# glgerard/MDBN

Hardware: AMD Instinct MI355X
Metric: CD-k Gibbs steps/sec (samples/sec), GRBM 4096->1024 CD-1 (higher is better)
Workload: dtype f32; 1 GPU; GRBM 4096->1024 CD-1, batch 512 per GPU, fp32, N(0,1) rows resident in HBM (BASELINE configs[1]); global_batch=512, k=1, n_data=32768, parallelism=dp1

## Files before the change

### include/mdbn_hip.h

```cpp
#ifndef MDBN_HIP_H
#define MDBN_HIP_H

#include <stddef.h>
#include <stdint.h>

#ifdef __cplusplus
extern "C" {
#endif

#define MDBN_OK       0
#define MDBN_EINVAL  (-1)
#define MDBN_EHIP    (-2)
#define MDBN_ENOSPC  (-3)

#define MDBN_VERSION 2

typedef struct mdbn_ctx mdbn_ctx;

typedef struct mdbn_rng {
    uint64_t seed;
    uint32_t stream_id;
    uint32_t step;
    uint32_t draw;
    uint32_t reserved;
// ... 49 lines not shown
    float batch_size;
    float n_rows;
    float cost_scale;
    float *cost_out;
    void *W_planes;
    int32_t phase;
    int32_t reserved;
} mdbn_update_args;

int  mdbn_version(void);
int  mdbn_last_error(char *buf, size_t n);
int  mdbn_source_hash(char *buf, size_t n);

int  mdbn_ctx_create(mdbn_ctx **out, int device);
int  mdbn_ctx_destroy(mdbn_ctx *ctx);

int  mdbn_bal_segment(int32_t tiles, int32_t stages, int32_t workgroups, int32_t w, int32_t k, int32_t *out);
int  mdbn_set_option(mdbn_ctx *ctx, const char *name, int64_t value);

int  mdbn_kernel_timing(mdbn_ctx *ctx, int enable);
int  mdbn_kernel_timing_read(mdbn_ctx *ctx, int64_t *n_launches, double *total_ms);
int  mdbn_kernel_timing_detail(mdbn_ctx *ctx, int64_t cap, double *ms, double *alg_flop,
                               double *pipe_flop, int32_t *kind, int64_t *n_launches);

int  mdbn_workspace_bytes(int64_t B, int64_t V, int64_t H, int64_t *bytes);
int  mdbn_workspace_bytes_ctx(mdbn_ctx *ctx, int64_t B, int64_t V, int64_t H, int64_t *bytes);
int  mdbn_padded_ld(int64_t cols, int64_t *ld);
int  mdbn_planes_bytes(int64_t B, int64_t ldv, int64_t ldh, int64_t *bytes);
int  mdbn_planes_alt_bytes(int64_t B, int64_t ldv, int64_t *bytes);
int  mdbn_ahead_bytes_ctx(mdbn_ctx *ctx, int64_t B, int64_t V, int64_t H, int64_t ldv, int64_t ldh, int64_t *bytes);
int  mdbn_planes_eligible(int64_t B, int64_t V, int64_t H, int64_t ldv, int64_t ldh, int32_t *eligible);
int  mdbn_planes_eligible_ctx(mdbn_ctx *ctx, int64_t B, int64_t V, int64_t H, int64_t ldv, int64_t ldh, int32_t *eligible);
int  mdbn_split_planes(mdbn_ctx *ctx, void *stream, const float *x, int64_t rows, int64_t ld, void *planes);
int  mdbn_stats_floats(int64_t V, int64_t ldv, int64_t ldh, int64_t *n);

int  mdbn_gather_rows(mdbn_ctx *ctx, void *stream, const float *src, int64_t n_rows,
                      int64_t cols, int64_t ld_src, const void *indexes, int index_is_64,
                      int64_t n_idx, float *dst, int64_t ld_dst);

int  mdbn_gather_rows_host(mdbn_ctx *ctx, void *stream, const float *src, int64_t n_rows,
                           int64_t cols, int64_t ld_src, const void *indexes, int index_is_64,
                           int64_t n_idx, float *dst, int64_t ld_dst, int workgroups, int threads);

int  mdbn_host_gather_rows(const float *table, int64_t n_rows, int64_t cols, int64_t ld,
                           const int64_t *indexes, int64_t n, float *out, int64_t ld_out, int threads);

// ... 193 lines not shown
```

### mdbn_amd/_lib.py

```python
import ctypes as C
import os

HERE = os.path.dirname(os.path.abspath(__file__))
LIB_PATH = os.path.join(HERE, "libmdbn_hip.so")


class MdbnError(RuntimeError):
    pass


class Rng(C.Structure):
    _fields_ = [("seed", C.c_uint64), ("stream_id", C.c_uint32), ("step", C.c_uint32),
                ("draw", C.c_uint32), ("reserved", C.c_uint32), ("row_offset", C.c_uint64)]


class _Sized(C.Structure):

    def __init__(self, *a, **kw):
        super(_Sized, self).__init__(*a, **kw)
        self.struct_size = C.sizeof(type(self))


class CdArgs(_Sized):
    _fields_ = [("struct_size", C.c_uint64), ("data", C.c_void_p), ("n_data", C.c_int64), ("indexes", C.c_void_p),
# ... 17 lines not shown
                ("vbias", C.c_void_p), ("vbias_speed", C.c_void_p),
                ("V", C.c_int64), ("H", C.c_int64), ("ldv", C.c_int64), ("ldh", C.c_int64),
                ("stats", C.c_void_p),
                ("lr", C.c_float), ("lambda_1", C.c_float), ("lambda_2", C.c_float),
                ("weightcost", C.c_float), ("momentum", C.c_float),
                ("batch_size", C.c_float), ("n_rows", C.c_float),
                ("cost_scale", C.c_float), ("cost_out", C.c_void_p), ("W_planes", C.c_void_p),
                ("phase", C.c_int32), ("reserved", C.c_int32)]


_i64, _i32, _f32, _vp = C.c_int64, C.c_int, C.c_float, C.c_void_p
_rngp = C.POINTER(Rng)

SIGNATURES = {
    "mdbn_version": [],
    "mdbn_last_error": [C.c_char_p, C.c_size_t],
    "mdbn_source_hash": [C.c_char_p, C.c_size_t],
    "mdbn_ctx_create": [C.POINTER(_vp), _i32],
    "mdbn_ctx_destroy": [_vp],
    "mdbn_set_option": [_vp, C.c_char_p, _i64],
    "mdbn_bal_segment": [_i32, _i32, _i32, _i32, _i32, C.POINTER(_i32)],
    "mdbn_kernel_timing": [_vp, _i32],
    "mdbn_kernel_timing_read": [_vp, C.POINTER(_i64), C.POINTER(C.c_double)],
    "mdbn_kernel_timing_detail": [_vp, _i64, C.POINTER(C.c_double), C.POINTER(C.c_double),
                                  C.POINTER(C.c_double), C.POINTER(C.c_int32), C.POINTER(_i64)],
    "mdbn_workspace_bytes": [_i64, _i64, _i64, C.POINTER(_i64)],
    "mdbn_workspace_bytes_ctx": [_vp, _i64, _i64, _i64, C.POINTER(_i64)],
    "mdbn_padded_ld": [_i64, C.POINTER(_i64)],
    "mdbn_planes_bytes": [_i64, _i64, _i64, C.POINTER(_i64)],
    "mdbn_planes_alt_bytes": [_i64, _i64, C.POINTER(_i64)],
    "mdbn_ahead_bytes_ctx": [_vp, _i64, _i64, _i64, _i64, _i64, C.POINTER(_i64)],
    "mdbn_planes_eligible": [_i64, _i64, _i64, _i64, _i64, C.POINTER(_i32)],
    "mdbn_planes_eligible_ctx": [_vp, _i64, _i64, _i64, _i64, _i64, C.POINTER(_i32)],
    "mdbn_split_planes": [_vp, _vp, _vp, _i64, _i64, _vp],
    "mdbn_stats_floats": [_i64, _i64, _i64, C.POINTER(_i64)],
    "mdbn_gather_rows": [_vp, _vp, _vp, _i64, _i64, _i64, _vp, _i32, _i64, _vp, _i64],
    "mdbn_gather_rows_host": [_vp, _vp, _vp, _i64, _i64, _i64, _vp, _i32, _i64, _vp, _i64, _i32, _i32],
    "mdbn_host_gather_rows": [_vp, _i64, _i64, _i64, _vp, _i64, _vp, _i64, _i32],
    "mdbn_feeder_create": [_vp, _vp, _i64, _i64, _i64, _i64, _i32, C.POINTER(_vp), _i64, _i32, C.POINTER(_vp)],
    "mdbn_feeder_submit": [_vp, _vp, _i64, C.POINTER(_i64)],
    "mdbn_feeder_acquire": [_vp, _i64, _vp, C.POINTER(_i32)],
    "mdbn_feeder_release": [_vp, _i64, _vp],
    "mdbn_feeder_stats": [_vp, C.POINTER(C.c_double)],
    "mdbn_feeder_cancel": [_vp],
    "mdbn_feeder_destroy": [_vp],
    "mdbn_propup_sample": [_vp, _vp, _vp, _i64, _i64, _vp, _i64, _i64, _i64, _vp,
# ... 125 lines not shown
```

### mdbn_amd/csrc/mdbn_capi.hip

```cpp
#include <hip/hip_runtime.h>
#include <algorithm>
#include <cstdint>
#include <initializer_list>
#include <cstdarg>
#include <cstdio>
#include <cstring>
#include <string>
#include <utility>
#include <vector>
#include "mdbn_capi_internal.h"
#include "mdbn_kernels.h"
#include "mdbn_small.h"
#include "mdbn_thin.h"
#include "mdbn_gchain.h"

using namespace mdbn;
using namespace mdbn::capi;

static const Options g_default_options;
static GemmTiming g_no_timing;
static thread_local const Options* t_opt = &g_default_options;
static thread_local GemmTiming* t_timing = &g_no_timing;
#define g_timing (*t_timing)

namespace mdbn {
namespace capi {
CtxScope::CtxScope(mdbn_ctx* c) : prev_opt(t_opt), prev_timing(t_timing)
{
// ... 82 lines not shown
    return p;
}

bool prefer_skinny(int64_t M, int64_t N, int64_t K)
{
    if (!g_opt_skinny_gemm) return false;
    if (M <= 64) return true;
    if (K > g_opt_skinny_fused_max_k) return false;
    const int64_t tiles_m = (M + 63) / 64, strips = (N + 31) / 32;
    if (K > 64 * tiles_m * strips) return false;
    return M * N * K <= (K <= 512 ? 3 : 1) * g_opt_skinny_max_macs;
}


#define g_opt_gemm_bf16x6 (t_opt->gemm_bf16x6)
#define g_opt_small_fused (t_opt->small_fused)
#define g_opt_thin_fused (t_opt->thin_fused)
#define g_opt_gchain (t_opt->gchain)
#define g_opt_gemm_planes (t_opt->gemm_planes)
#define g_opt_planes_mfma (t_opt->planes_mfma)
#define g_opt_early_w (t_opt->early_w)
#define g_opt_narrow_tiles (t_opt->narrow_tiles)
#define g_opt_slab_tail (t_opt->slab_tail)
#define g_opt_feed_copy_streams (t_opt->feed_copy_streams)
#define g_opt_gather_ahead (t_opt->gather_ahead)
#define g_opt_bf16_inputs (t_opt->bf16_inputs)
#define g_opt_planes_min_work (t_opt->planes_min_work)
#define g_opt_comm_cus (t_opt->comm_cus)
#define g_opt_bal_blocks (t_opt->bal_blocks)
constexpr int kMaxBalBlocks = 256;

bool try_bf16x6(Plan& p, int64_t M, int64_t N, int64_t K, bool unsplit = false)
{
    if (p.skinny || K < 64) return false;
    const int64_t tm = (M + 127) / 128, tn = (N + 127) / 128, tiles = tm * tn;
    int64_t sk = 1;
    if (!unsplit) {
        sk = std::min(std::max<int64_t>(1, kTargetJobs / tiles), std::max<int64_t>(1, K / kMinSplitK));
    } else if (p.splitk != 1) {
        return false;
    }
    if (tiles * sk < g_opt_x6_min_jobs) return false;
    int64_t kchunk = ((K + sk - 1) / sk + 31) / 32 * 32;
    sk = (K + kchunk - 1) / kchunk;
    p.x6 = 1;
    p.bn = 128; p.bk = 32; p.cw = 1;
// ... 220 lines not shown
                      const unsigned short* Wp, int64_t V, int64_t H, int64_t ncols, int64_t rows, EpiArgs e, bool want_cost,
                      const Workspace& ws, hipStream_t s, int* n_cost_out)
{
    const int64_t Kdim = dir == 0 ? V : H, Ndim = dir == 0 ? H : V;
    PlaneGemmArgs g{};
    g.A = A; g.lda = lda; g.pa = pa; g.ap = ap;
    g.B = Wp; g.ldb = H; g.pb = V * H;
    g.M = (int)rows; g.N = (int)Ndim; g.K = (int)Kdim;
    g.tiles_m = (int)(rows / 128); g.tiles_n = (int)(Ndim / 128);
    {
        const Plan p = plan_forward(rows, Ndim, Kdim, e.ld, false);
        g.splitk = p.splitk; g.kchunk = p.kchunk;
    }
    int bal = bal_blocks(ctx, comm_cus, (int64_t)g.tiles_m * g.tiles_n, Kdim / 32), bal_slabs = 0;
    if (bal) {
        bal_slabs = bal_max_segments(g.tiles_m * g.tiles_n, (int)(Kdim / 32), bal);
        if ((int64_t)bal_slabs * rows * e.ld > ws.slab_floats) bal = 0;
        if ((int64_t)bal_slabs * rows * e.ld * 4 >= (int64_t)1 << 31) bal = 0;
    }
    if (!bal && g_opt_narrow_tiles && g_opt_fused_epilogue && dir == 1 && g.splitk == 2 && Ndim % 64 == 0 && g_opt_planes_mfma == 16 &&
        !g_opt_bf16_inputs && (ap == 1 || ap == 3) && (int64_t)g.tiles_m * (Ndim / 64) <= 2 * ctx->num_cu &&
        (!e.target || (e.ld_target % 4 == 0 && ((uintptr_t)e.target & 15) == 0))) {
        g.bn = 64; g.tiles_n = (int)(Ndim / 64); g.splitk = 1; g.kchunk = (int)Kdim;
    }
    const bool fuse = !bal && g_opt_fused_epilogue && g.splitk == 1;
    const int nb = fuse ? g.tiles_m * g.tiles_n : epilogue_blocks(rows, e.ld);
    e.rows = (int)rows; e.cols = (int)ncols;
    e.cost_partials = nullptr;
    if (want_cost) {
        if (nb > ws.cost_floats) return fail(MDBN_ENOSPC, "cost scratch exhausted");
        e.cost_partials = ws.cost_partials;
        if (n_cost_out) *n_cost_out = nb;
    }
    const int lb = dir == 0 ? LAY_MN : LAY_K;
    if (bal) {
        g.bal = bal; g.fused = 0; g.C = ws.slabs; g.ldc = e.ld; g.slab_stride = rows * e.ld;
        g.xcd_group = bal >= 4 * g.tiles_m * g.tiles_n ? 0 : 1;
        g.splitk = 1; g.kchunk = (int)Kdim; g.c_bytes = (int64_t)bal_slabs * rows * e.ld * 4;
        e.slabs = ws.slabs; e.slab_stride = g.slab_stride; e.nsplit = bal_slabs;
        e.bal_P = bal; e.bal_S = (int)(Kdim / 32); e.bal_tiles_m = g.tiles_m; e.bal_tiles_n = g.tiles_n;
        {
            const int tiles = g.tiles_m * g.tiles_n;
            bool uniform = true;
            for (int t = 0; t < tiles && uniform; ++t) uniform = bal_tile_slabs(t, tiles, e.bal_S, bal) == bal_slabs;
            if (uniform) e.bal_P = 0;
        }
// ... 366 lines not shown
    return MDBN_OK;
}

int mdbn_last_error(char* buf, size_t n)
{
    if (!buf || n == 0) return MDBN_EINVAL;
    snprintf(buf, n, "%s", g_err.c_str());
    return MDBN_OK;
}

int mdbn_ctx_create(mdbn_ctx** out, int device)
{
    REQUIRE(out != nullptr, "out is NULL");
    int count = 0;
    HIP_OK(hipGetDeviceCount(&count));
    REQUIRE(device >= 0 && device < count, "device %d out of range (%d visible)", device, count);
    hipDeviceProp_t prop;
    HIP_OK(hipGetDeviceProperties(&prop, device));
    if (strncmp(prop.gcnArchName, "gfx950", 6) != 0)
        return fail(MDBN_EHIP, "device %d is %s; this library is built for gfx950 only", device, prop.gcnArchName);
    mdbn_ctx* c = new mdbn_ctx;
    c->device = device;
    c->num_cu = prop.multiProcessorCount;
    *out = c;
    return MDBN_OK;
}

int mdbn_ctx_destroy(mdbn_ctx* ctx)
{
    CtxScope ctx_scope(ctx);
    if (ctx) {
        if (ctx->ev_fork) (void)hipEventDestroy(ctx->ev_fork);
        if (ctx->ev_join) (void)hipEventDestroy(ctx->ev_join);
        if (ctx->side) (void)hipStreamDestroy(ctx->side);
        if (ctx->comm) (void)mdbn_comm_destroy(ctx);
        if (ctx->gc_flags) (void)hipFree(ctx->gc_flags);
    }
    delete ctx;
    return MDBN_OK;
}

#ifdef MDBN_STAMP
int mdbn_debug_set_stamps(void* p) { g_stamps = (unsigned long long*)p; return MDBN_OK; }
#endif

int mdbn_bal_segment(int32_t tiles, int32_t stages, int32_t workgroups, int32_t w, int32_t k, int32_t* out)
// ... 162 lines not shown
        return MDBN_OK;
    }
    if (strcmp(name, "fused_update") == 0) {
        ctx->opt.fused_update = value != 0;
        return MDBN_OK;
    }
    if (strcmp(name, "fused_epilogue") == 0) {
        ctx->opt.fused_epilogue = value != 0;
        return MDBN_OK;
    }
    if (strcmp(name, "update_overlap") == 0) {
        ctx->opt.update_overlap = value != 0;
        return MDBN_OK;
    }
    return fail(MDBN_EINVAL, "unknown option %s", name);
}

int mdbn_kernel_timing(mdbn_ctx* ctx, int enable)
{
    CtxScope ctx_scope(ctx);
    REQUIRE(ctx != nullptr, "ctx is NULL");
    g_timing.enabled = enable != 0;
    g_timing.used = 0;
    return MDBN_OK;
}

int mdbn_kernel_timing_read(mdbn_ctx* ctx, int64_t* n_launches, double* total_ms)
{
    CtxScope ctx_scope(ctx);
    REQUIRE(ctx && n_launches && total_ms, "NULL argument");
    double tot = 0.0;
    for (size_t i = 0; i < g_timing.used; ++i) {
        HIP_OK(hipEventSynchronize(g_timing.pool[i].second));
        float ms = 0.f;
        HIP_OK(hipEventElapsedTime(&ms, g_timing.pool[i].first, g_timing.pool[i].second));
        tot += ms;
    }
    *n_launches = (int64_t)g_timing.used;
    *total_ms = tot;
    return MDBN_OK;
}

int mdbn_kernel_timing_detail(mdbn_ctx* ctx, int64_t cap, double* ms, double* alg_flop, double* pipe_flop,
                              int32_t* kind, int64_t* n_launches)
{
    CtxScope ctx_scope(ctx);
// ... 809 lines not shown
```

### mdbn_amd/csrc/mdbn_capi_internal.h

```cpp
#pragma once
#include <hip/hip_runtime.h>
#include <cstdint>
#include <utility>
#include <vector>
#include "mdbn_kernels.h"

namespace mdbn {
namespace capi {

struct Options {
    int gemm_bk = 0;
    int x6_min_jobs = 48;
    int x6_pw = 4;
    int gemm_cw = 0;
    int update_overlap = 0;
    int fused_epilogue = 1;
    int fused_update = 1;
    int fused_finalize = 1;
    int skinny_gemm = 1;
    int skinny_fused_max_k = 1024;
    int64_t skinny_max_macs = 32ll << 20;
    int stream_x6 = 2;
    int64_t stream_max_macs = (int64_t)1 << 30;
    int stream_mi = 0;
    int stream_ni = 0;
    int gemm_bf16x6 = 3;
    int small_fused = 1;
    int thin_fused = 1;
    int gchain = 0;
    int gemm_planes = 1;
    int planes_mfma = 16;
    int early_w = 1;
    int narrow_tiles = 1;
    int slab_tail = 1;
    int feed_copy_streams = 1;
    int gather_ahead = 1;
    int bf16_inputs = 0;
    int64_t planes_min_work = (int64_t)1 << 30;
    int comm_cus = 0;
    int bal_blocks = 0;
    int min_splitk = 128;
    int epilogue_cw = 0;
    int epilogue_threads = 0;
    int small_fin_lanes = 0;
};

struct GemmTiming {
    bool enabled = false;
    std::vector<std::pair<hipEvent_t, hipEvent_t>> pool;
    struct Meta { int kind; double alg_flop, pipe_flop; };
    std::vector<Meta> meta;
    size_t used = 0;
};

}
}

struct mdbn_ctx {
    int device;
    int num_cu;
    mdbn::capi::Options opt;
    mdbn::capi::GemmTiming timing;
    int pending_n_cost = -1;
    const void* pending_stats = nullptr;
    void* comm = nullptr;
    int comm_ranks = 0;
    hipStream_t side = nullptr;
    hipEvent_t ev_fork = nullptr, ev_join = nullptr;
    unsigned* gc_flags = nullptr;
    unsigned gc_seq = 1;
};

namespace mdbn {
namespace capi {

struct CtxScope {
    const Options* prev_opt; GemmTiming* prev_timing;
    explicit CtxScope(mdbn_ctx* c);
    ~CtxScope();
    CtxScope(const CtxScope&) = delete;
    CtxScope& operator=(const CtxScope&) = delete;
};

int fail(int code, const char* fmt, ...) __attribute__((format(printf, 2, 3)));

// ... 65 lines not shown
```

### mdbn_amd/csrc/mdbn_kernels.h

```cpp
#pragma once
#include <hip/hip_runtime.h>
#include <stdint.h>
#include "philox.h"
#include "../../include/mdbn_hip.h"

namespace mdbn {

enum { LAY_K = 0, LAY_MN = 1 };

struct EpiArgs {
    const float* slabs;
    int64_t slab_stride;
    int nsplit;
    int rows, cols;
    int64_t ld;
    const float* bias;
    float* pre;
    float* mean;
    float* sample;
    float mean_scale;
    int gauss;
    const float* target;
    int64_t ld_target;
    const void* target_idx;
// ... 81 lines not shown
    int B, rpw, passes;
    unsigned short* P; int64_t plane_stride, ld;
};

struct PlaneGemmArgs {
    const unsigned short* A; int64_t lda, pa;
    const unsigned short* B; int64_t ldb, pb;
    float* C; int64_t ldc, slab_stride;
    int M, N, K, kchunk, splitk, tiles_m, tiles_n;
    int ap;
    int ms;
    int bn;
    int fused;
    int slab_tail;
    unsigned long long* stamps;
    int bal;
    int xcd_group;
    float* scratch;
    int64_t c_bytes;
    EpiArgs epi;
    UpdEpi upd;
    int fin_enabled;
    int stats_tail;
    FinArgs fin;
    GatherAhead ga;
    DeferredBias db;
};

__host__ __device__ inline int bal_first_unit(int w, int P, int64_t U) { return (int)(((int64_t)w * U) / P); }
__host__ __device__ inline int bal_block_of(int64_t u, int P, int64_t U) { return (int)(((u + 1) * P - 1) / U); }
__host__ __device__ inline int bal_rem_blocks(int tiles, int S, int P)
{
    const int64_t Ur = (int64_t)(tiles - (tiles / P) * P) * S;
    return Ur < P ? (int)Ur : P;
}
__host__ __device__ inline int bal_tile_slabs(int t, int tiles, int S, int P)
{
    const int Tf = (tiles / P) * P;
    if (t < Tf) return 1;
    const int64_t Ur = (int64_t)(tiles - Tf) * S, u0 = (int64_t)(t - Tf) * S;
    const int Pr = bal_rem_blocks(tiles, S, P);
    return bal_block_of(u0 + S - 1, Pr, Ur) - bal_block_of(u0, Pr, Ur) + 1;
}
hipError_t launch_gemm_planes(int la, int lb, const PlaneGemmArgs& g, hipStream_t s);
bool slab_tail_ok(const PlaneGemmArgs& g, int la, int lb);
bool stats_tail_ok(const PlaneGemmArgs& g, int la, int lb);
hipError_t launch_gemm_planes_bal(int la, int lb, const PlaneGemmArgs& g, hipStream_t s);
int bal_max_segments(int tiles, int stages, int P);
int bal_segment_host(int tiles, int S, int P, int w, int k, int* tile, int* s0, int* s1, int* nseg, int* nt);
hipError_t launch_split_planes(const float* X, int64_t rows, int64_t ld, unsigned short* P, int64_t plane_stride, hipStream_t s);
hipError_t launch_gather_planes(const float* src, int64_t n_rows, int64_t cols_ld, int64_t ld_src, const void* idx, int idx64,
                                int64_t n_idx, float* dst, int64_t ld_dst, unsigned short* P, int64_t plane_stride, hipStream_t s);

int epilogue_blocks(int64_t rows, int64_t ld);
int epilogue_cw(int64_t rows, int64_t ld);
void set_epilogue_cw(int cw);
void set_epilogue_threads(int t);
inline int row_groups(int64_t B) { return (int)((B + 3) / 4); }

hipError_t launch_gemm(int la, int lb, const GemmArgs& g, hipStream_t s);
hipError_t launch_act_epilogue(const EpiArgs& e, hipStream_t s);
hipError_t launch_sum_slabs(const float* slabs, int nsplit, int64_t slab_stride, int64_t n,
                            float* out, hipStream_t s);
hipError_t launch_gather_slim(const float* src, int64_t n_rows, int64_t cols_ld, int64_t ld_src, const void* idx, int idx64,
                              int64_t n_idx, float* dst, int64_t ld_dst, int blocks, int threads, hipStream_t s);
hipError_t launch_gather(const float* src, int64_t n_rows, int64_t cols_ld, int64_t ld_src,
                         const void* idx, int idx64, int64_t n_idx, float* dst, int64_t ld_dst,
                         hipStream_t s);
hipError_t launch_colsum_groups(const float* X, const float* Y, int rows, int64_t ld, float* out, hipStream_t s);
// ... 24 lines not shown
```

### mdbn_amd/csrc/mdbn_planes.hip

```cpp
#include <hip/hip_runtime.h>
#include <algorithm>
#include <stdint.h>
#include "mdbn_kernels.h"
#include "mdbn_device.h"

namespace mdbn {

typedef __bf16 pbf16x8 __attribute__((ext_vector_type(8)));
typedef short ps16x4 __attribute__((ext_vector_type(4)));
typedef short ps16x8 __attribute__((ext_vector_type(8)));
typedef float pf32x16 __attribute__((ext_vector_type(16)));
typedef float pf32x4 __attribute__((ext_vector_type(4)));
typedef unsigned int pu32x4b __attribute__((ext_vector_type(4)));
typedef unsigned int pu32x2b __attribute__((ext_vector_type(2)));

#ifndef PL_ARGS_EARLY
#define PL_ARGS_EARLY 1
#endif
#ifndef PL_SIDE_WT
#define PL_SIDE_WT 0
#endif
constexpr int PL_PLANE = 8192, PL_STAGE = 6 * PL_PLANE, PL_NSTAGE = 3, PL_LW = 4;

__device__ __forceinline__ void pl_glds16(const void* g, unsigned lds_off, char* smem)
{
    __builtin_amdgcn_global_load_lds((const __attribute__((address_space(1))) void*)g,
                                     (__attribute__((address_space(3))) void*)(smem + lds_off), 16, 0, 0);
// ... 22 lines not shown
            g.stamps[(int64_t)blockIdx.x * 16 + (SLOT)] = wall_clock64();                     \
    } while (0)
#else
#define PL_STAMP(SLOT) do {} while (0)
#endif
struct EarlySpeed { float4 sp[16], w0[16]; };
__device__ __forceinline__ void deferred_bias_update(const DeferredBias& d, int wave, int lane)
{
    for (int64_t i = (int64_t)blockIdx.x * 256 + wave * 64 + lane; i < d.H + d.V; i += (int64_t)gridDim.x * 256) {
        if (i < d.H) {
            const float sn = upd_speed(upd_scale(d.s_h[i], d.inv_rows), d.hbs[i], d.mu);
            d.hbs[i] = sn;
            d.hb[i] = upd_param(d.hb[i], 1.0f, sn, d.lr);
        } else {
            const int64_t j = i - d.H;
            const float sn = upd_speed(upd_scale(d.s_v[j], d.inv_rows), d.vbs[j], d.mu);
            d.vbs[j] = sn;
            d.vb[j] = upd_param(d.vb[j], 1.0f, sn, d.lr);
        }
    }
    if (blockIdx.x == 0 && wave == 0 && lane == 0 && d.cost_out) d.cost_out[0] = d.cost_sum[0] * d.cost_scale;
}

template <int LA, int LB, int AP, int MS, bool EARLYW = false, int BN = 128>
__device__ __forceinline__ void pl_loader(const PlaneGemmArgs& g, char* smem, int w, int lane, int m0, int n0, int kbeg, int nt,
                                          EarlySpeed* es = nullptr)
{
    PL_STAMP(0);
    static_assert(BN == 128 || (BN == 64 && LB == LAY_K), "a 64-column tile is implemented for a ROW B operand");
    constexpr int NA = AP == 3 ? 3 : 1, NB = AP == 0 ? 1 : 3;
    constexpr int QB = BN / 16;
    constexpr int NQ = 8 * NA + QB * NB, PER = NQ / PL_LW;
    static_assert(NQ % PL_LW == 0, "staging instructions must divide over the loader waves");
    const char* src[PER];
    unsigned dst[PER];
    int64_t step[PER];
#pragma unroll
    for (int j = 0; j < PER; ++j) {
        const int q = w + j * PL_LW;
        const bool isA = q < 8 * NA;
        const int plane = isA ? q / 8 : (q - 8 * NA) / QB, sub = isA ? (q & 7) : (q - 8 * NA) % QB;
        const int lay = isA ? LA : LB;
        const unsigned short* base = isA ? g.A + plane * g.pa : g.B + plane * g.pb;
        const int64_t ld = isA ? g.lda : g.ldb;
        const int mn0 = isA ? m0 : n0;
        dst[j] = (isA ? plane : 3 + plane) * PL_PLANE + sub * 1024;
        if (lay == LAY_K) {
            const int row = 16 * sub + (lane >> 2);
            const int c = (lane & 3) ^ pl_row_swz<MS>(row);
            src[j] = reinterpret_cast<const char*>(base + (int64_t)(mn0 + row) * ld + kbeg + 8 * c);
            step[j] = 64;
        } else {
            const int k = 4 * sub + (lane >> 4);
            const int ch = (lane & 15) ^ pl_col_swz<MS>(k);
            src[j] = reinterpret_cast<const char*>(base + (int64_t)(kbeg + k) * ld + mn0 + 8 * ch);
            step[j] = 64 * ld;
        }
    }
#define PL_ISSUE(T)                                                                           \
    do {                                                                                      \
        const unsigned so = ((T) % PL_NSTAGE) * PL_STAGE;                                     \
        _Pragma("unroll") for (int j = 0; j < PER; ++j) {                                     \
// ... 384 lines not shown
    (void)bar_wait;
    int offA[4][2], offB[4][2];
    pl_offsets16<LA, LB>(lane, wm, wn, offA, offB);
    PL_CONSUME_CONSTS();
    pbf16x8 Alo[3][2], Ahi[3][2], Blo[3][2], Bhi[3][2];
    if (open_barrier) __syncthreads();
    RD_A(Alo, smem, 0);
    RD_B(Blo, smem, 0);
    for (int it = 0; it < nt; it += 2) {
        {
            const char* base = smem + (it % PL_NSTAGE) * PL_STAGE;
            const char* next = smem + ((it + 1) % PL_NSTAGE) * PL_STAGE;
            PL_STAGE_EVEN(base, next, PL_MAIN_BARRIER());
        }
        if (it + 1 < nt) {
            const char* base = smem + ((it + 1) % PL_NSTAGE) * PL_STAGE;
            const char* next = smem + ((it + 2) % PL_NSTAGE) * PL_STAGE;
            PL_STAGE_ODD(base, next, PL_MAIN_BARRIER());
        }
    }
    if (bar_wait_out) *bar_wait_out = bar_wait;
}

template <int LA, int LB, int AP, int FUSED, int MS, int BN = 128>
__global__ __launch_bounds__(64 * (4 + PL_LW)) void gemm_planes_kernel(PlaneGemmArgs g)
{
    static_assert(BN == 128 || (BN == 64 && MS == 16 && FUSED == 1 && LB == LAY_K), "64-column tiles: unsplit ROW-operand forward pass");
    extern __shared__ __attribute__((aligned(16))) char smem[];
#if PL_ARGS_EARLY
    asm volatile("" :: "s"(g.A), "s"(g.lda), "s"(g.pa), "s"(g.B), "s"(g.ldb), "s"(g.pb), "s"(g.C), "s"(g.ldc), "s"(g.slab_stride),
                 "s"(g.kchunk), "s"(g.tiles_m), "s"(g.tiles_n), "s"((int)gridDim.x));
#endif
    const int nwg = gridDim.x, bid = blockIdx.x;
    const int xcd = bid & 7, slot = bid >> 3;
    const int qq = nwg >> 3, rem = nwg & 7;
    const int w = (xcd < rem ? xcd * (qq + 1) : rem * (qq + 1) + (xcd - rem) * qq) + slot;
    const int tiles = g.tiles_m * g.tiles_n;
    const int ks = w / tiles, t = w - ks * tiles;
    int tm, tn;
    if (g.tiles_m <= g.tiles_n) { tn = t / g.tiles_m; tm = t - tn * g.tiles_m; }
    else { tm = t / g.tiles_n; tn = t - tm * g.tiles_n; }
    const int m0 = tm * 128, n0 = tn * BN;
    const int kbeg = ks * g.kchunk;
    const int nt = g.kchunk / 32;
    const int wave = __builtin_amdgcn_readfirstlane(threadIdx.x >> 6);
    const int lane = threadIdx.x & 63;

    EarlySpeed es;
    (void)es;
    if (wave >= 4) {
        pl_loader<LA, LB, AP, MS, (FUSED == 2 || (FUSED == 0 && LA == LAY_MN && LB == LAY_MN && AP == 3)) && MS == 16, BN>(
            g, smem, wave - 4, lane, m0, n0, kbeg, nt, &es);
        if constexpr (FUSED == 0) return;
    } else {
        const int r = lane & 31, h = lane >> 5;
        const int wm = (wave >> 1) * 64, wn = (wave & 1) * (BN / 2);
        if constexpr (FUSED == 0 && LA == LAY_MN && LB == LAY_MN) {
            if (g.db.on) deferred_bias_update(g.db, wave, lane);
        }
        if constexpr ((FUSED == 2 || FUSED == 0) && LA == LAY_MN && LB == LAY_MN) {
            if (g.fin_enabled) {
                const int nu = fin_units(g.fin);
                for (int unit = wave * (int)gridDim.x + (int)blockIdx.x; unit <= nu; unit += 4 * (int)gridDim.x)
                    finalize_unit(g.fin, unit, lane);
            }
        }
        if constexpr (MS == 16) {
            constexpr int NBH = BN / 64, NBB = 2 * NBH;
            pf32x4a acc[4][NBB];
#pragma unroll
            for (int a = 0; a < 4; ++a)
#pragma unroll
                for (int b = 0; b < NBB; ++b) acc[a][b] = pf32x4a{0.f, 0.f, 0.f, 0.f};
#ifdef MDBN_STAMP
#define PL_MSTAMP(SLOT)                                                                       \
    do {                                                                                      \
        if (PL_STAMP_COND && g.stamps && wave == 0 && lane == 0)                              \
            g.stamps[(int64_t)blockIdx.x * 16 + (SLOT)] = wall_clock64();                     \
    } while (0)
#else
#define PL_MSTAMP(SLOT) do {} while (0)
#endif
            PL_MSTAMP(8);
            __syncthreads();
            PL_MSTAMP(9);
#ifdef MDBN_STAMP
            if (PL_STAMP_COND && g.stamps && wave == 0 && lane == 0)
                g.stamps[(int64_t)blockIdx.x * 16 + 13] = clock64();
#endif
#ifdef MDBN_STAMP
            long long bw = 0;
            pl_consume16<LA, LB, AP, NBH>(smem, nt, lane, wm, wn, acc, false, &bw);
#else
            pl_consume16<LA, LB, AP, NBH>(smem, nt, lane, wm, wn, acc, false);
#endif
            PL_MSTAMP(10);
#ifdef MDBN_STAMP
            if (PL_STAMP_COND && g.stamps && wave == 0 && lane == 0) {
                g.stamps[(int64_t)blockIdx.x * 16 + 14] = clock64();
                g.stamps[(int64_t)blockIdx.x * 16 + 15] = bw;
            }
#endif
            const int c16 = lane & 15, q4 = lane >> 4;
            if constexpr (FUSED != 0) {
                float* T = reinterpret_cast<float*>(smem);
                constexpr int LDT = BN + 8;
#pragma unroll
                for (int a = 0; a < 4; ++a)
#pragma unroll
                    for (int b = 0; b < NBB; ++b)
#pragma unroll
                        for (int e = 0; e < 4; ++e)
                            T[(wm + 16 * a + 4 * q4 + e) * LDT + wn + 16 * b + c16] = acc[a][b][e];
            } else {
                float* C = g.C + (int64_t)ks * g.slab_stride;
#pragma unroll
                for (int a = 0; a < 4; ++a)
// ... 162 lines not shown
                constexpr int LDT = 128 + 8;
#pragma unroll
                for (int j = 0; j < 16; ++j) {
                    const int row = 8 * j + (lt >> 5), c4 = lt & 31;
                    const float4 st = *reinterpret_cast<const float4*>(T + row * LDT + 4 * c4);
                    float4 sn;
#pragma unroll
                    for (int c = 0; c < 4; ++c)
                        setc(sn, c, upd_speed(upd_grad(comp(st, c), g.upd.inv_bs, g.upd.wc, comp(es.w0[j], c)), comp(es.sp[j], c), g.upd.mu));
                    *reinterpret_cast<float4*>(g.upd.Ws + (int64_t)(m0 + row) * g.upd.ld + n0 + 4 * c4) = sn;
                }
            }
        }
        else fused_update_epilogue<128, 128, NT>(g.upd, T, m0, n0);
#ifdef MDBN_STAMP
        if (PL_STAMP_COND && g.stamps && threadIdx.x == 0) {
            asm volatile("s_waitcnt vmcnt(0)" ::: "memory");
            g.stamps[(int64_t)blockIdx.x * 16 + 12] = wall_clock64();
        }
#endif
    }
}

template <int LA, int LB, int AP, int FUSED, int MS, int BN = 128>
static hipError_t launch_planes_m(const PlaneGemmArgs& g, hipStream_t s)
{
    auto kern = gemm_planes_kernel<LA, LB, AP, FUSED, MS, BN>;
    static bool attr_set = false;
    constexpr int lds = PL_NSTAGE * PL_STAGE;
    if (!attr_set) {
        hipError_t e = hipFuncSetAttribute(reinterpret_cast<const void*>(kern), hipFuncAttributeMaxDynamicSharedMemorySize, lds);
        if (e != hipSuccess) return e;
        attr_set = true;
    }
    hipLaunchKernelGGL(kern, dim3(g.tiles_m * g.tiles_n * g.splitk), dim3(64 * (4 + PL_LW)), lds, s, g);
    return hipGetLastError();
}

template <int LA, int LB, int AP, int FUSED>
static hipError_t launch_planes_t(const PlaneGemmArgs& g, hipStream_t s)
{
    if constexpr (AP == 0) return launch_planes_m<LA, LB, 0, FUSED, 16>(g, s);
    else return g.ms == 32 ? launch_planes_m<LA, LB, AP, FUSED, 32>(g, s) : launch_planes_m<LA, LB, AP, FUSED, 16>(g, s);
}

#ifndef PL_TAIL_T
#define PL_TAIL_T 2
#endif
#ifndef PL_TAIL_WT
#define PL_TAIL_WT 1
// ... 259 lines not shown
        hipError_t e = hipFuncSetAttribute(reinterpret_cast<const void*>(kern), hipFuncAttributeMaxDynamicSharedMemorySize, lds);
        if (e != hipSuccess) return e;
        attr_set = true;
    }
    hipLaunchKernelGGL(kern, dim3(g.tiles_m * g.tiles_n), dim3(64 * (4 + PL_LW)), lds, s, g);
    return hipGetLastError();
}

bool stats_tail_ok(const PlaneGemmArgs& g, int la, int lb)
{
    const int nt = g.kchunk / 32;
    return la == LAY_MN && lb == LAY_MN && g.ap == 3 && g.fused == 2 && g.upd.early == 1 && g.ms == 16 && g.bn != 64 && !g.bal &&
           g.splitk == 1 && nt >= 12 && (nt & 1) == 0 && (g.upd.ld & 3) == 0 && g.upd.ld < ((int64_t)1 << 21) &&
           (reinterpret_cast<uintptr_t>(g.upd.Ws) & 15) == 0;
}

bool slab_tail_ok(const PlaneGemmArgs& g, int la, int lb)
{
    return la == LAY_K && lb == LAY_MN && (g.ap == 1 || g.ap == 3) && g.fused == 0 && g.ms == 16 && g.bn != 64 && !g.bal &&
           (g.ldc & 3) == 0 && (g.slab_stride & 3) == 0 && (reinterpret_cast<uintptr_t>(g.C) & 15) == 0 &&
           (int64_t)g.M * g.ldc * 4 < ((int64_t)1 << 31);
}

hipError_t launch_gemm_planes(int la, int lb, const PlaneGemmArgs& g, hipStream_t s)
{
    if (g.bn == 64) {
        if (g.M % 128 || g.N % 64 || g.K % 32 || g.kchunk != g.K || g.splitk != 1 || g.tiles_m != g.M / 128 || g.tiles_n != g.N / 64 ||
            (g.lda & 7) || (g.ldb & 7) || g.fused != 1 || la != LAY_K || lb != LAY_K || g.ms != 16 || (g.ap != 1 && g.ap != 3))
            return hipErrorInvalidValue;
        return g.ap == 1 ? launch_planes_m<LAY_K, LAY_K, 1, 1, 16, 64>(g, s) : launch_planes_m<LAY_K, LAY_K, 3, 1, 16, 64>(g, s);
    }
    if (g.M % 128 || g.N % 128 || g.kchunk % 32 || g.kchunk * g.splitk != g.K || g.tiles_m != g.M / 128 ||
        g.tiles_n != g.N / 128 || (g.lda & 7) || (g.ldb & 7) || ((g.fused == 1 || g.fused == 2) && g.splitk != 1) ||
        (g.ap != 0 && g.ap != 1 && g.ap != 3))
        return hipErrorInvalidValue;
    if (g.slab_tail) {
        if (!slab_tail_ok(g, la, lb)) return hipErrorInvalidValue;
        return g.ap == 1 ? launch_planes_slabtail<1>(g, s) : launch_planes_slabtail<3>(g, s);
    }
    if (g.stats_tail) {
        if (!stats_tail_ok(g, la, lb)) return hipErrorInvalidValue;
#if PL_STATS_TAIL
        return launch_planes_statstail(g, s);
#endif
    }
#define PL_CASE(LAV, LBV, APV, FV) \
    if (la == LAV && lb == LBV && g.ap == APV && g.fused == FV) return launch_planes_t<LAV, LBV, APV, FV>(g, s)
    PL_CASE(LAY_K, LAY_MN, 3, 0); PL_CASE(LAY_K, LAY_MN, 3, 1); PL_CASE(LAY_K, LAY_MN, 1, 0); PL_CASE(LAY_K, LAY_MN, 1, 1);
    PL_CASE(LAY_K, LAY_K, 3, 0); PL_CASE(LAY_K, LAY_K, 3, 1); PL_CASE(LAY_K, LAY_K, 1, 0); PL_CASE(LAY_K, LAY_K, 1, 1);
    PL_CASE(LAY_MN, LAY_MN, 3, 0); PL_CASE(LAY_MN, LAY_MN, 3, 2);
    PL_CASE(LAY_K, LAY_MN, 0, 0); PL_CASE(LAY_K, LAY_MN, 0, 1); PL_CASE(LAY_K, LAY_K, 0, 0); PL_CASE(LAY_K, LAY_K, 0, 1);
    PL_CASE(LAY_MN, LAY_MN, 0, 0); PL_CASE(LAY_MN, LAY_MN, 0, 2);
// ... 442 lines not shown
```

### mdbn_amd/engine.py

```python
import ctypes as C
import os as _os
from collections import namedtuple

import numpy
import torch

from . import _lib


def round_up4(n):
    return (int(n) + 3) & ~3


def padded_ld(cols):
    return round_up4(cols)


_default_engine = None


def get_engine():
    global _default_engine
    if _default_engine is None:
        _default_engine = HipEngine()
# ... 1081 lines not shown
        for t in tensors:
            base = t._base if t._base is not None else t
            _lib.check(self.lib.mdbn_count_nonfinite(self.ctx, self._stream(), self._p(base), base.numel(),
                                                     self._p(count)), "mdbn_count_nonfinite")
        return int(count.item())

    def rng_uniform(self, rows, cols, rng, normal=False):
        out = self.alloc_matrix(rows, cols)
        r = rng.c()
        fn = self.lib.mdbn_rng_normal if normal else self.lib.mdbn_rng_uniform
        _lib.check(fn(self.ctx, self._stream(), self._p(out), rows, cols, out.stride(0), C.byref(r)),
                   "mdbn_rng_*")
        return out

    def kernel_timing(self, enable):
        _lib.check(self.lib.mdbn_kernel_timing(self.ctx, int(bool(enable))), "mdbn_kernel_timing")

    def kernel_timing_read(self):
        n, ms = C.c_int64(), C.c_double()
        _lib.check(self.lib.mdbn_kernel_timing_read(self.ctx, C.byref(n), C.byref(ms)),
                   "mdbn_kernel_timing_read")
        return n.value, ms.value

    def kernel_timing_detail(self, cap=8192):
        ms, alg, pipe = (C.c_double * cap)(), (C.c_double * cap)(), (C.c_double * cap)()
        kind, n = (C.c_int32 * cap)(), C.c_int64()
        _lib.check(self.lib.mdbn_kernel_timing_detail(self.ctx, cap, ms, alg, pipe, kind, C.byref(n)),
                   "mdbn_kernel_timing_detail")
        m = min(cap, n.value)
        return [(ms[i], alg[i], pipe[i], kind[i]) for i in range(m)]

    def narrow_bf16(self, src, out=None):
        if out is None or out.numel() != src.numel():
            out = torch.empty(src.numel(), dtype=torch.bfloat16, device=self.device)
        _lib.check(self.lib.mdbn_f32_to_bf16(self.ctx, self._stream(), self._p(src), C.c_void_p(out.data_ptr()), src.numel()),
                   "mdbn_f32_to_bf16")
        return out

    def widen_bf16(self, wire, dst):
        _lib.check(self.lib.mdbn_bf16_to_f32(self.ctx, self._stream(), C.c_void_p(wire.data_ptr()), self._p(dst), dst.numel()),
                   "mdbn_bf16_to_f32")
        return dst

    def cost_values(self, costs):
        out, blocks = [0.0] * len(costs), {}
        for i, c in enumerate(costs):
# ... 11 lines not shown
```

Baseline: 3.976 million samples/s.

## Add 64-deep K stages for the narrow one-plane planes GEMM

Adds a variant of the narrow 64-column planes GEMM that stages K in 64-wide slices with a swizzled LDS image. The consumer double-buffers fragments and interleaves LDS reads with MFMA through sched_group_barrier hints. The aim is to halve pipeline iterations and barriers per tile and improve MFMA issue density on the forward pass. It is on by default, can be disabled with an env var, and counts its launches through a new API. The cost is larger stage buffers and more register pressure.

```diff
diff --git a/include/mdbn_hip.h b/include/mdbn_hip.h
--- a/include/mdbn_hip.h
+++ b/include/mdbn_hip.h
@@ -95,6 +95,7 @@
 int  mdbn_kernel_timing_read(mdbn_ctx *ctx, int64_t *n_launches, double *total_ms);
 int  mdbn_kernel_timing_detail(mdbn_ctx *ctx, int64_t cap, double *ms, double *alg_flop,
                                double *pipe_flop, int32_t *kind, int64_t *n_launches);
+int  mdbn_narrow_deep_launches(mdbn_ctx *ctx, int64_t *n_launches);
 
 int  mdbn_workspace_bytes(int64_t B, int64_t V, int64_t H, int64_t *bytes);
 int  mdbn_workspace_bytes_ctx(mdbn_ctx *ctx, int64_t B, int64_t V, int64_t H, int64_t *bytes);
diff --git a/mdbn_amd/_lib.py b/mdbn_amd/_lib.py
--- a/mdbn_amd/_lib.py
+++ b/mdbn_amd/_lib.py
@@ -63,6 +63,7 @@
     "mdbn_bal_segment": [_i32, _i32, _i32, _i32, _i32, C.POINTER(_i32)],
     "mdbn_kernel_timing": [_vp, _i32],
     "mdbn_kernel_timing_read": [_vp, C.POINTER(_i64), C.POINTER(C.c_double)],
+    "mdbn_narrow_deep_launches": [_vp, C.POINTER(_i64)],
     "mdbn_kernel_timing_detail": [_vp, _i64, C.POINTER(C.c_double), C.POINTER(C.c_double),
                                   C.POINTER(C.c_double), C.POINTER(C.c_int32), C.POINTER(_i64)],
     "mdbn_workspace_bytes": [_i64, _i64, _i64, C.POINTER(_i64)],
diff --git a/mdbn_amd/csrc/mdbn_capi.hip b/mdbn_amd/csrc/mdbn_capi.hip
--- a/mdbn_amd/csrc/mdbn_capi.hip
+++ b/mdbn_amd/csrc/mdbn_capi.hip
@@ -4,6 +4,7 @@
 #include <initializer_list>
 #include <cstdarg>
 #include <cstdio>
+#include <cstdlib>
 #include <cstring>
 #include <string>
 #include <utility>
@@ -132,6 +133,7 @@
 #define g_opt_early_w (t_opt->early_w)
 #define g_opt_narrow_tiles (t_opt->narrow_tiles)
 #define g_opt_slab_tail (t_opt->slab_tail)
+#define g_opt_narrow_deep (t_opt->narrow_deep)
 #define g_opt_feed_copy_streams (t_opt->feed_copy_streams)
 #define g_opt_gather_ahead (t_opt->gather_ahead)
 #define g_opt_bf16_inputs (t_opt->bf16_inputs)
@@ -398,6 +400,9 @@
         !g_opt_bf16_inputs && (ap == 1 || ap == 3) && (int64_t)g.tiles_m * (Ndim / 64) <= 2 * ctx->num_cu &&
         (!e.target || (e.ld_target % 4 == 0 && ((uintptr_t)e.target & 15) == 0))) {
         g.bn = 64; g.tiles_n = (int)(Ndim / 64); g.splitk = 1; g.kchunk = (int)Kdim;
+        g.fused = 1; g.ms = 16;
+        g.deep = g_opt_narrow_deep && narrow_deep_ok(g, LAY_K, LAY_K);
+        if (g.deep) ++ctx->narrow_deep_launches;
     }
     const bool fuse = !bal && g_opt_fused_epilogue && g.splitk == 1;
     const int nb = fuse ? g.tiles_m * g.tiles_n : epilogue_blocks(rows, e.ld);
@@ -810,6 +815,7 @@
     mdbn_ctx* c = new mdbn_ctx;
     c->device = device;
     c->num_cu = prop.multiProcessorCount;
+    if (const char* e = getenv("MDBN_NARROW_DEEP")) c->opt.narrow_deep = atoi(e) != 0;
     *out = c;
     return MDBN_OK;
 }
@@ -1018,6 +1024,13 @@
     REQUIRE(ctx != nullptr, "ctx is NULL");
     g_timing.enabled = enable != 0;
     g_timing.used = 0;
+    return MDBN_OK;
+}
+
+int mdbn_narrow_deep_launches(mdbn_ctx* ctx, int64_t* n_launches)
+{
+    REQUIRE(ctx && n_launches, "NULL argument");
+    *n_launches = ctx->narrow_deep_launches;
     return MDBN_OK;
 }
 
diff --git a/mdbn_amd/csrc/mdbn_capi_internal.h b/mdbn_amd/csrc/mdbn_capi_internal.h
--- a/mdbn_amd/csrc/mdbn_capi_internal.h
+++ b/mdbn_amd/csrc/mdbn_capi_internal.h
@@ -33,6 +33,7 @@
     int early_w = 1;
     int narrow_tiles = 1;
     int slab_tail = 1;
+    int narrow_deep = 1;
     int feed_copy_streams = 1;
     int gather_ahead = 1;
     int bf16_inputs = 0;
@@ -61,6 +62,7 @@
     int num_cu;
     mdbn::capi::Options opt;
     mdbn::capi::GemmTiming timing;
+    int64_t narrow_deep_launches = 0;
     int pending_n_cost = -1;
     const void* pending_stats = nullptr;
     void* comm = nullptr;
diff --git a/mdbn_amd/csrc/mdbn_kernels.h b/mdbn_amd/csrc/mdbn_kernels.h
--- a/mdbn_amd/csrc/mdbn_kernels.h
+++ b/mdbn_amd/csrc/mdbn_kernels.h
@@ -127,6 +127,7 @@
     UpdEpi upd;
     int fin_enabled;
     int stats_tail;
+    int deep;
     FinArgs fin;
     GatherAhead ga;
     DeferredBias db;
@@ -150,6 +151,7 @@
 hipError_t launch_gemm_planes(int la, int lb, const PlaneGemmArgs& g, hipStream_t s);
 bool slab_tail_ok(const PlaneGemmArgs& g, int la, int lb);
 bool stats_tail_ok(const PlaneGemmArgs& g, int la, int lb);
+bool narrow_deep_ok(const PlaneGemmArgs& g, int la, int lb);
 hipError_t launch_gemm_planes_bal(int la, int lb, const PlaneGemmArgs& g, hipStream_t s);
 int bal_max_segments(int tiles, int stages, int P);
 int bal_segment_host(int tiles, int S, int P, int w, int k, int* tile, int* s0, int* s1, int* nseg, int* nt);
diff --git a/mdbn_amd/csrc/mdbn_planes.hip b/mdbn_amd/csrc/mdbn_planes.hip
--- a/mdbn_amd/csrc/mdbn_planes.hip
+++ b/mdbn_amd/csrc/mdbn_planes.hip
@@ -3,6 +3,7 @@
 #include <stdint.h>
 #include "mdbn_kernels.h"
 #include "mdbn_device.h"
+#include "mdbn_planes_image.h"
 
 namespace mdbn {
 
@@ -71,7 +72,7 @@
     if (blockIdx.x == 0 && wave == 0 && lane == 0 && d.cost_out) d.cost_out[0] = d.cost_sum[0] * d.cost_scale;
 }
 
-template <int LA, int LB, int AP, int MS, bool EARLYW = false, int BN = 128>
+template <int LA, int LB, int AP, int MS, bool EARLYW = false, int BN = 128, int KD = 32>
 __device__ __forceinline__ void pl_loader(const PlaneGemmArgs& g, char* smem, int w, int lane, int m0, int n0, int kbeg, int nt,
                                           EarlySpeed* es = nullptr)
 {
@@ -79,7 +80,9 @@
     static_assert(BN == 128 || (BN == 64 && LB == LAY_K), "a 64-column tile is implemented for a ROW B operand");
     constexpr int NA = AP == 3 ? 3 : 1, NB = AP == 0 ? 1 : 3;
     constexpr int QB = BN / 16;
-    constexpr int NQ = 8 * NA + QB * NB, PER = NQ / PL_LW;
+    static_assert(KD == 32 || (KD == 64 && AP == 1 && BN == 64 && LA == LAY_K && LB == LAY_K && MS == 16 && !EARLYW),
+                  "64-deep stages: the narrow one-plane ROW x ROW kernel");
+    constexpr int NQ = KD == 64 ? deep_image::NQ : 8 * NA + QB * NB, PER = NQ / PL_LW;
     static_assert(NQ % PL_LW == 0, "staging instructions must divide over the loader waves");
     const char* src[PER];
     unsigned dst[PER];
@@ -87,6 +90,15 @@
 #pragma unroll
     for (int j = 0; j < PER; ++j) {
         const int q = w + j * PL_LW;
+        if constexpr (KD == 64) {
+            const deep_image::Piece pc = deep_image::loader_piece(q, lane);
+            const unsigned short* base = pc.is_a ? g.A : g.B + pc.plane * g.pb;
+            dst[j] = deep_image::instr_base(q);
+            src[j] = reinterpret_cast<const char*>(base + (int64_t)((pc.is_a ? m0 : n0) + pc.row) * (pc.is_a ? g.lda : g.ldb) + kbeg +
+                                                   8 * pc.src_chunk);
+            step[j] = 2 * KD;
+            continue;
+        }
         const bool isA = q < 8 * NA;
         const int plane = isA ? q / 8 : (q - 8 * NA) / QB, sub = isA ? (q & 7) : (q - 8 * NA) % QB;
         const int lay = isA ? LA : LB;
@@ -517,10 +529,68 @@
     if (bar_wait_out) *bar_wait_out = bar_wait;
 }
 
-template <int LA, int LB, int AP, int FUSED, int MS, int BN = 128>
+template <int AP>
+__device__ __forceinline__ void pl_consume16_deep(char* smem, int nt, int lane, int wm, int wn, pf32x4a (&acc)[4][2],
+                                                  long long* bar_wait_out = nullptr)
+{
+    static_assert(AP == 1, "64-deep stages hold one plane of A (three would need 72 KB a slot)");
+    long long bar_wait = 0;
+    (void)bar_wait;
+    int offA[4][2], offB[2][2];
+#pragma unroll
+    for (int kh = 0; kh < 2; ++kh) {
+#pragma unroll
+        for (int b = 0; b < 4; ++b) offA[b][kh] = deep_image::plane_base(true, 0) + deep_image::frag_offset(wm + 16 * b, kh, lane);
+#pragma unroll
+        for (int b = 0; b < 2; ++b) offB[b][kh] = deep_image::frag_offset(wn + 16 * b, kh, lane);
+    }
+    pbf16x8 A0[4], B0[3][2], A1[4], B1[3][2];
+#define DP_RD(FA, FB, BASE, KH)                                                               \
+    do {                                                                                      \
+        _Pragma("unroll") for (int b = 0; b < 4; ++b) FA[b] = *reinterpret_cast<const pbf16x8*>((BASE) + offA[b][KH]); \
+        _Pragma("unroll") for (int pl = 0; pl < 3; ++pl)                                      \
+            _Pragma("unroll") for (int b = 0; b < 2; ++b)                                     \
+                FB[pl][b] = *reinterpret_cast<const pbf16x8*>((BASE) + deep_image::plane_base(false, pl) + offB[b][KH]); \
+    } while (0)
+#define DP_MM(FA, FB)                                                                         \
+    _Pragma("unroll") for (int pl = 2; pl >= 0; --pl)                                         \
+        _Pragma("unroll") for (int a = 0; a < 4; ++a)                                         \
+            _Pragma("unroll") for (int b = 0; b < 2; ++b)                                     \
+                acc[a][b] = __builtin_amdgcn_mfma_f32_16x16x32_bf16(FA[a], FB[pl][b], acc[a][b], 0, 0, 0);
+#define DP_ORD()                                                                              \
+    _Pragma("unroll") for (int i_ = 0; i_ < 10; ++i_) {                                       \
+        __builtin_amdgcn_sched_group_barrier(0x100, 1, 0);                                    \
+        __builtin_amdgcn_sched_group_barrier(0x008, 1, 0);                                    \
+    }                                                                                         \
+    __builtin_amdgcn_sched_group_barrier(0x008, 14, 0);
+#define DP_PIN(FA, FB)                                                                        \
+    do {                                                                                      \
+        _Pragma("unroll") for (int b = 0; b < 4; ++b) asm volatile("" :: "v"(FA[b]));         \
+        _Pragma("unroll") for (int pl = 0; pl < 3; ++pl)                                      \
+            _Pragma("unroll") for (int b = 0; b < 2; ++b) asm volatile("" :: "v"(FB[pl][b])); \
+    } while (0)
+    DP_RD(A0, B0, smem, 0);
+    for (int it = 0; it < nt; ++it) {
+        const char* base = smem + (it % PL_NSTAGE) * PL_STAGE;
+        const char* next = smem + ((it + 1) % PL_NSTAGE) * PL_STAGE;
+        DP_RD(A1, B1, base, 1); DP_MM(A0, B0); DP_ORD();
+        __builtin_amdgcn_sched_barrier(0);
+        DP_PIN(A1, B1);
+        PL_MAIN_BARRIER();
+        DP_RD(A0, B0, next, 0); DP_MM(A1, B1); DP_ORD();
+    }
+#undef DP_RD
+#undef DP_MM
+#undef DP_ORD
+#undef DP_PIN
+    if (bar_wait_out) *bar_wait_out = bar_wait;
+}
+
+template <int LA, int LB, int AP, int FUSED, int MS, int BN = 128, int KD = 32>
 __global__ __launch_bounds__(64 * (4 + PL_LW)) void gemm_planes_kernel(PlaneGemmArgs g)
 {
     static_assert(BN == 128 || (BN == 64 && MS == 16 && FUSED == 1 && LB == LAY_K), "64-column tiles: unsplit ROW-operand forward pass");
+    static_assert(KD == 32 || (KD == 64 && BN == 64 && AP == 1 && LA == LAY_K), "64-deep stages: narrow one-plane forward pass");
     extern __shared__ __attribute__((aligned(16))) char smem[];
 #if PL_ARGS_EARLY
     asm volatile("" :: "s"(g.A), "s"(g.lda), "s"(g.pa), "s"(g.B), "s"(g.ldb), "s"(g.pb), "s"(g.C), "s"(g.ldc), "s"(g.slab_stride),
@@ -537,14 +607,14 @@
     else { tm = t / g.tiles_n; tn = t - tm * g.tiles_n; }
     const int m0 = tm * 128, n0 = tn * BN;
     const int kbeg = ks * g.kchunk;
-    const int nt = g.kchunk / 32;
+    const int nt = g.kchunk / KD;
     const int wave = __builtin_amdgcn_readfirstlane(threadIdx.x >> 6);
     const int lane = threadIdx.x & 63;
 
     EarlySpeed es;
     (void)es;
     if (wave >= 4) {
-        pl_loader<LA, LB, AP, MS, (FUSED == 2 || (FUSED == 0 && LA == LAY_MN && LB == LAY_MN && AP == 3)) && MS == 16, BN>(
+        pl_loader<LA, LB, AP, MS, (FUSED == 2 || (FUSED == 0 && LA == LAY_MN && LB == LAY_MN && AP == 3)) && MS == 16, BN, KD>(
             g, smem, wave - 4, lane, m0, n0, kbeg, nt, &es);
         if constexpr (FUSED == 0) return;
     } else {
@@ -585,9 +655,11 @@
 #endif
 #ifdef MDBN_STAMP
             long long bw = 0;
-            pl_consume16<LA, LB, AP, NBH>(smem, nt, lane, wm, wn, acc, false, &bw);
+            if constexpr (KD == 64) pl_consume16_deep<AP>(smem, nt, lane, wm, wn, acc, &bw);
+            else pl_consume16<LA, LB, AP, NBH>(smem, nt, lane, wm, wn, acc, false, &bw);
 #else
-            pl_consume16<LA, LB, AP, NBH>(smem, nt, lane, wm, wn, acc, false);
+            if constexpr (KD == 64) pl_consume16_deep<AP>(smem, nt, lane, wm, wn, acc);
+            else pl_consume16<LA, LB, AP, NBH>(smem, nt, lane, wm, wn, acc, false);
 #endif
             PL_MSTAMP(10);
 #ifdef MDBN_STAMP
@@ -796,10 +868,10 @@
     }
 }
 
-template <int LA, int LB, int AP, int FUSED, int MS, int BN = 128>
+template <int LA, int LB, int AP, int FUSED, int MS, int BN = 128, int KD = 32>
 static hipError_t launch_planes_m(const PlaneGemmArgs& g, hipStream_t s)
 {
-    auto kern = gemm_planes_kernel<LA, LB, AP, FUSED, MS, BN>;
+    auto kern = gemm_planes_kernel<LA, LB, AP, FUSED, MS, BN, KD>;
     static bool attr_set = false;
     constexpr int lds = PL_NSTAGE * PL_STAGE;
     if (!attr_set) {
@@ -1105,12 +1177,27 @@
            (int64_t)g.M * g.ldc * 4 < ((int64_t)1 << 31);
 }
 
+#ifndef PL_NARROW_DEEP
+#define PL_NARROW_DEEP 1
+#endif
+bool narrow_deep_ok(const PlaneGemmArgs& g, int la, int lb)
+{
+    return PL_NARROW_DEEP && g.bn == 64 && la == LAY_K && lb == LAY_K && g.ap == 1 && g.fused == 1 && g.ms == 16 && !g.bal &&
+           g.splitk == 1 && g.kchunk == g.K && g.K % 128 == 0 && g.K >= 256 && g.lda % 64 == 0 && g.ldb % 64 == 0 && g.pb % 64 == 0;
+}
+
 hipError_t launch_gemm_planes(int la, int lb, const PlaneGemmArgs& g, hipStream_t s)
 {
     if (g.bn == 64) {
         if (g.M % 128 || g.N % 64 || g.K % 32 || g.kchunk != g.K || g.splitk != 1 || g.tiles_m != g.M / 128 || g.tiles_n != g.N / 64 ||
             (g.lda & 7) || (g.ldb & 7) || g.fused != 1 || la != LAY_K || lb != LAY_K || g.ms != 16 || (g.ap != 1 && g.ap != 3))
             return hipErrorInvalidValue;
+        if (g.deep) {
+            if (!narrow_deep_ok(g, la, lb)) return hipErrorInvalidValue;
+#if PL_NARROW_DEEP
+            return launch_planes_m<LAY_K, LAY_K, 1, 1, 16, 64, 64>(g, s);
+#endif
+        }
         return g.ap == 1 ? launch_planes_m<LAY_K, LAY_K, 1, 1, 16, 64>(g, s) : launch_planes_m<LAY_K, LAY_K, 3, 1, 16, 64>(g, s);
     }
     if (g.M % 128 || g.N % 128 || g.kchunk % 32 || g.kchunk * g.splitk != g.K || g.tiles_m != g.M / 128 ||
diff --git a/mdbn_amd/csrc/mdbn_planes_image.h b/mdbn_amd/csrc/mdbn_planes_image.h
--- /dev/null
+++ b/mdbn_amd/csrc/mdbn_planes_image.h
@@ -0,0 +1,55 @@
+#pragma once
+
+#if defined(__HIPCC__)
+#define MDBN_IMG_FN __host__ __device__ inline
+#else
+#define MDBN_IMG_FN inline
+#endif
+
+namespace mdbn {
+namespace deep_image {
+
+constexpr int KD = 64;
+constexpr int ROW_BYTES = 2 * KD;
+constexpr int A_ROWS = 128, W_ROWS = 64, W_PLANES = 3;
+constexpr int A_BYTES = A_ROWS * ROW_BYTES, W_BYTES = W_ROWS * ROW_BYTES;
+constexpr int STAGE_BYTES = A_BYTES + W_PLANES * W_BYTES;
+constexpr int INSTR_ROWS = 8, INSTR_BYTES = INSTR_ROWS * ROW_BYTES;
+constexpr int A_INSTR = A_ROWS / INSTR_ROWS, W_INSTR = W_ROWS / INSTR_ROWS;
+constexpr int NQ = A_INSTR + W_PLANES * W_INSTR;
+
+MDBN_IMG_FN int swz(int row) { return (row >> 1) & 7; }
+
+MDBN_IMG_FN int plane_base(bool is_a, int plane) { return is_a ? 0 : A_BYTES + plane * W_BYTES; }
+
+struct Piece {
+    bool is_a;
+    int plane;
+    int row;
+    int src_chunk;
+    int lds;
+};
+MDBN_IMG_FN int instr_base(int q)
+{
+    return q < A_INSTR ? q * INSTR_BYTES : plane_base(false, (q - A_INSTR) / W_INSTR) + ((q - A_INSTR) % W_INSTR) * INSTR_BYTES;
+}
+MDBN_IMG_FN Piece loader_piece(int q, int lane)
+{
+    Piece p;
+    p.is_a = q < A_INSTR;
+    p.plane = p.is_a ? 0 : (q - A_INSTR) / W_INSTR;
+    const int sub = p.is_a ? q : (q - A_INSTR) % W_INSTR;
+    p.row = INSTR_ROWS * sub + (lane >> 3);
+    p.src_chunk = (lane & 7) ^ swz(p.row);
+    p.lds = instr_base(q) + 16 * lane;
+    return p;
+}
+
+MDBN_IMG_FN int frag_offset(int row0, int kh, int lane)
+{
+    const int row = row0 + (lane & 15), c = 4 * kh + (lane >> 4);
+    return row * ROW_BYTES + ((c ^ swz(row)) << 4);
+}
+
+}
+}
diff --git a/mdbn_amd/engine.py b/mdbn_amd/engine.py
--- a/mdbn_amd/engine.py
+++ b/mdbn_amd/engine.py
@@ -1127,6 +1127,11 @@
                    "mdbn_kernel_timing_read")
         return n.value, ms.value
 
+    def narrow_deep_launches(self):
+        n = C.c_int64()
+        _lib.check(self.lib.mdbn_narrow_deep_launches(self.ctx, C.byref(n)), "mdbn_narrow_deep_launches")
+        return n.value
+
     def kernel_timing_detail(self, cap=8192):
         ms, alg, pipe = (C.c_double * cap)(), (C.c_double * cap)(), (C.c_double * cap)()
         kind, n = (C.c_int32 * cap)(), C.c_int64()
```

Result: faster. 4.019 million samples/s, median of 6 (+1.1%).
